# CHIANGEL/MAP-CODE

Measured on AMD Instinct MI355X. Metric: pretrain samples/sec (DCNv2+MFP, Avazu, bs4096), higher is better.
Workload: dtype f32; 1 GPU; DCNv2+MFP pretrain step, avazu-shaped synthetic ids (Zipf(1.1) per field), F=23, V=9449445, E=16, H=1000x3, cross x3, P=32, K=25, mask_ratio 0.3, fp32 GEMMs as three fp16 MFMAs per product (operands scaled by per-tensor magnitude records and cut into two fp16 pieces, fp32 accumulation; weights cut once per optimizer step); per_gpu_batch=4096, global_batch=4096, parallelism=dp1, launch=hipGraph replay of the whole step, table_optimizer=row-sparse AdamW with lazy replay of untouched rows, 400 untimed pre-roll steps

## Files before the change

### map-code_amd/csrc/amax.h

```cpp
#pragma once
#include "common.h"

namespace mapx {

typedef unsigned long long amax_rec;
constexpr int kAmaxSlots = 64;

const int32_t* amax_epoch_ptr();

__device__ inline uint32_t finite_abs_bits(float v) {
  const uint32_t u = __float_as_uint(v) & 0x7fffffffu;
  return u < 0x7f800000u ? u : 0u;
}
__device__ inline uint32_t amax4(uint32_t m, float a, float b, float c, float d) {
  const uint32_t x = max(finite_abs_bits(a), finite_abs_bits(b)), y = max(finite_abs_bits(c), finite_abs_bits(d));
  return max(m, max(x, y));
}
__device__ inline uint32_t wave_max_u32(uint32_t v) {
#pragma unroll
  for (int o = 32; o >= 1; o >>= 1) v = max(v, (uint32_t)__shfl_xor((int)v, o, kWave));
  return v;
}
__device__ inline int amax_slot() {
  return (int)(((blockIdx.x + blockIdx.y * gridDim.x + blockIdx.z * gridDim.x * gridDim.y) * (blockDim.x >> 6) +
                (threadIdx.x >> 6)) & (kAmaxSlots - 1));
}
__device__ inline void amax_publish(amax_rec* rec, uint32_t bits, const int32_t* epoch, int ahead = 0, int slot = 0) {
  const unsigned long long tag = epoch ? (unsigned long long)(uint32_t)(*epoch + ahead) : 0ull;
  atomicMax(rec + (slot & (kAmaxSlots - 1)), (tag << 32) | bits);
}
__device__ inline void amax_publish_wave(amax_rec* rec, uint32_t bits, const int32_t* epoch, int ahead = 0) {
  bits = wave_max_u32(bits);
  if ((threadIdx.x & 63) == 0) amax_publish(rec, bits, epoch, ahead, amax_slot());
}

__device__ inline void amax_publish_block(amax_rec* rec, uint32_t bits, const int32_t* epoch, int ahead = 0) {
  __shared__ uint32_t wave_bits[16];
  bits = wave_max_u32(bits);
  if ((threadIdx.x & 63) == 0) wave_bits[threadIdx.x >> 6] = bits;
  __syncthreads();
  if (threadIdx.x == 0) {
    uint32_t m = wave_bits[0];
    for (int w = 1; w < (int)(blockDim.x >> 6); ++w) m = max(m, wave_bits[w]);
    amax_publish(rec, m, epoch, ahead, (int)(blockIdx.x + blockIdx.y * gridDim.x + blockIdx.z * gridDim.x * gridDim.y));
  }
  __syncthreads();
}

__device__ inline uint32_t amax_read(const float* rec) {
  if (!rec) return 0u;
  return wave_max_u32(reinterpret_cast<const uint32_t*>(rec)[2 * (threadIdx.x & 63)] & 0x7fffffffu);
}
__device__ inline int h2_scale_exp(const float* rec) {
  const uint32_t b = amax_read(rec);
  const int e = (int)(b >> 23);
  if (b == 0u || e == 255) return 0;
  int n = 14 - (e - 127);
  return n > 126 ? 126 : (n < -126 ? -126 : n);
}
__device__ inline float pow2f(int n) { return __uint_as_float((uint32_t)(n + 127) << 23); }

}
```

### map-code_amd/csrc/gemm.hip

```cpp
#include "../../include/mapx_hip.h"
#include "common.h"
#include "amax.h"
#include "gemm_grouped.h"
#include "gemm_x3_common.h"

namespace mapx {


constexpr int kLayoutMaxT = 96 * 1024;

constexpr int kLayoutMwThreads = 1024;
constexpr int kLayoutBatch = 8;
__global__ void __launch_bounds__(kLayoutMwThreads) enc_group_layout_mw_kernel(
    const int64_t* __restrict__ masked_index, int T, int L, int F, int cap_slots, int32_t* __restrict__ rowmap,
    int32_t* __restrict__ hpos, int32_t* __restrict__ tile_group, int32_t* __restrict__ group_start) {
  constexpr int NW = kLayoutMwThreads / 64;
  __shared__ int hist[64];
  __shared__ int wave_match[NW];
  __shared__ int gs[64 + 1];
  extern __shared__ uint8_t fld[];
  const int f = blockIdx.x;
  const int lane = threadIdx.x & 63, wave = threadIdx.x >> 6;
  if (threadIdx.x < 64) hist[threadIdx.x] = 0;
  __syncthreads();
// ... 282 lines not shown
}

extern "C" int mapx_gemm_f32_batched(int count, int a_kc, int b_kc, int M, int N, int K, const float* const* A,
                                     int64_t lda, const float* const* B, int64_t ldb, float* const* C, int nsplit,
                                     void* ws, size_t ws_bytes, const mapx_gemm_scale* scales_opt,
                                     hipStream_t stream) {
  using namespace mapx;
  MAPX_REQUIRE(count >= 1 && count <= 4 && A && B && C, "gemm_f32_batched: 1 to 4 problems");
  MAPX_REQUIRE(M > 0 && N > 0 && K > 0, "gemm_f32_batched: empty problem");
  MAPX_REQUIRE(!(a_kc == 0 && b_kc != 0), "gemm_f32_batched: layout (A m-contiguous, B k-contiguous) unused");
  if (nsplit < 1) nsplit = 1;
  GemmX3Extra ex{};
  ex.batch = count;
  for (int z = 0; z < count; ++z) {
    MAPX_REQUIRE(A[z] && B[z] && C[z], "gemm_f32_batched: null operand");
    ex.Az[z] = A[z]; ex.Bz[z] = B[z]; ex.Cz[z] = C[z];
    if (scales_opt) { ex.amax_az[z] = scales_opt[z].amax_a; ex.amax_bz[z] = scales_opt[z].amax_b; }
  }
  if (count == 1) {
    ex.amax_a = ex.amax_az[0]; ex.amax_b = ex.amax_bz[0];
    return gemm_f32x3_launch(a_kc, b_kc, M, N, K, A[0], lda, B[0], ldb, C[0], N, MAPX_EPI_NONE, nullptr, nullptr, 0,
                             nullptr, 0, nullptr, 0, nsplit, -1, ws, ws_bytes, nullptr, stream, &ex);
  }
  int got = 0;
  for (int z = 1; z < count; ++z)
    MAPX_REQUIRE(((uintptr_t)A[z] % 16 == 0) == ((uintptr_t)A[0] % 16 == 0) &&
                     ((uintptr_t)B[z] % 16 == 0) == ((uintptr_t)B[0] % 16 == 0),
                 "gemm_f32_batched: operands of one launch must share their alignment");
  const int st = gemm_f32x3_launch(a_kc, b_kc, M, N, K, A[0], lda, B[0], ldb, C[0], N, MAPX_EPI_NONE, nullptr, nullptr, 0,
                                   nullptr, 0, nullptr, 0, nsplit, -1, ws, ws_bytes, &got, stream, &ex);
  if (st != MAPX_OK) return st;
  if (got > 1) {
    SumTasks t;
    memset(&t, 0, sizeof(t));
    for (int z = 0; z < count; ++z) {
      t.t[z].dst = C[z];
      t.t[z].src = static_cast<const float*>(ws) + (int64_t)z * nsplit * M * N;
      t.t[z].stride = (int64_t)M * N; t.t[z].n = (int64_t)M * N; t.t[z].nsplit = got;
    }
    hipLaunchKernelGGL(sum_tasks_kernel, dim3(96, count), dim3(256), 0, stream, t);
  }
  return check_launch("gemm_f32_batched");
}

extern "C" int mapx_enc_group_layout(const int64_t* masked_index, int T, int L, int F, int cap_slots,
                                     int32_t* rowmap, int32_t* hpos, int32_t* tile_group,
                                     int32_t* group_start, hipStream_t stream) {
  using namespace mapx;
  MAPX_REQUIRE(masked_index && rowmap && hpos && tile_group && group_start, "enc_group_layout: null pointer");
  MAPX_REQUIRE(F >= 1 && F <= 64 && L >= 1 && T >= 0 && cap_slots % 128 == 0 && cap_slots >= T + 127 * F,
               "enc_group_layout: bad sizes (F <= 64, cap_slots multiple of 128 and >= T + 127 F)");
  MAPX_REQUIRE(T <= kLayoutMaxT, "enc_group_layout: at most %d targets per step", kLayoutMaxT);
  const size_t dyn = ((size_t)T + 15) & ~(size_t)15;
  static bool raised = false;
  if (!raised) {
    MAPX_HIP(hipFuncSetAttribute(reinterpret_cast<const void*>(&enc_group_layout_mw_kernel),
                                 hipFuncAttributeMaxDynamicSharedMemorySize, kLayoutMaxT));
    raised = true;
  }
  hipLaunchKernelGGL(enc_group_layout_mw_kernel, dim3(F), dim3(kLayoutMwThreads), dyn, stream, masked_index, T, L, F,
                     cap_slots, rowmap, hpos, tile_group, group_start);
  return check_launch("enc_group_layout");
}

extern "C" int mapx_enc_grouped_fwd(const float* final_act, int64_t ld_final, int nrows, int K, const float* W,
                                    int64_t ldw, const float* bias, const int32_t* rowmap,
                                    const int32_t* tile_group, const int32_t* group_start_opt, int F,
                                    int cap_slots, float* h_slots, float* zero_slots_opt,
                                    const mapx_gemm_scale* scale_opt, hipStream_t stream) {
  using namespace mapx;
  MAPX_REQUIRE(final_act && W && bias && rowmap && tile_group && h_slots, "enc_grouped_fwd: null pointer");
  MAPX_REQUIRE(K % 4 == 0 && ld_final % 4 == 0 && ldw % 4 == 0 && cap_slots % 128 == 0,
               "enc_grouped_fwd: K, leading dimensions %% 4 and cap_slots %% 128 must be 0");
  GroupedArgs g{};
  g.A = final_act; g.lda = ld_final; g.B = W; g.ldb = ldw; g.C = h_slots; g.ldc = 32; g.bias = bias;
  g.rowmap = rowmap; g.tile_group = tile_group; g.K = K; g.N = 32; g.nrows = nrows;
  g.group_start = group_start_opt; g.F = F;
  g.zero_out = zero_slots_opt;
  MAPX_REQUIRE(K % 8 == 0 && ld_final % 4 == 0 && ldw % 4 == 0 && (uintptr_t)final_act % 16 == 0 && (uintptr_t)W % 16 == 0,
               "enc_grouped_fwd: K %% 8 != 0 or operands not 16-byte aligned (use the dense encoder GEMM)");
  static const bool h2 = [] { const char* e = getenv("MAPX_GEMM_H2"); return !e || atoi(e) != 0; }();
  if (h2 && scale_opt && scale_opt->amax_a && scale_opt->amax_b) {
    g.amax_a = scale_opt->amax_a; g.amax_b = scale_opt->amax_b;
    MAPX_HIP(enc_grouped_fwd_h2_launch(g, cap_slots, stream));
  } else {
    MAPX_HIP(enc_grouped_fwd_x3_launch(g, cap_slots, stream));
  }
  return check_launch("enc_grouped_fwd");
}

extern "C" int mapx_enc_grouped_dw(const float* dh_slots, const float* final_act, int64_t ld_final, int nrows,
                                   int N, const int32_t* rowmap, const int32_t* group_start, int F,
                                   const float* gscale_opt, float* dW, int64_t ldw, const mapx_gemm_scale* scale_opt,
                                   hipStream_t stream) {
  using namespace mapx;
  MAPX_REQUIRE(dh_slots && final_act && rowmap && group_start && dW, "enc_grouped_dw: null pointer");
  MAPX_REQUIRE(N % 4 == 0 && ld_final % 4 == 0 && F >= 1, "enc_grouped_dw: N, ld %% 4 must be 0");
  GroupedArgs g{};
  g.A = dh_slots; g.lda = 32; g.B = final_act; g.ldb = ld_final; g.C = dW; g.ldc = ldw;
  g.rowmap = rowmap; g.group_start = group_start; g.F = F; g.K = 0; g.N = N; g.nrows = nrows;
  g.gscale = gscale_opt;
  MAPX_REQUIRE(N % 8 == 0 && (uintptr_t)final_act % 16 == 0 && (uintptr_t)dh_slots % 16 == 0,
               "enc_grouped_dw: N %% 8 != 0 or operands not 16-byte aligned (use the dense encoder GEMM)");
  static const bool h2 = [] { const char* e = getenv("MAPX_GEMM_H2"); return !e || atoi(e) != 0; }();
  if (h2 && scale_opt && scale_opt->amax_a && scale_opt->amax_b) {
    g.amax_a = scale_opt->amax_a; g.amax_b = scale_opt->amax_b;
    MAPX_HIP(enc_grouped_dw_h2_launch(g, F, stream));
  } else {
    MAPX_HIP(enc_grouped_dw_x3_launch(g, F, stream));
  }
  return check_launch("enc_grouped_dw");
}

extern "C" size_t mapx_colsum_workspace_bytes(int N) {
  return (size_t)mapx::kColChunks * N * sizeof(float);
}

extern "C" int mapx_sum_tasks(const mapx_sum_task* tasks_host, int ntasks, hipStream_t stream) {
  using namespace mapx;
  MAPX_REQUIRE(ntasks >= 0 && ntasks <= kMaxSumTasks, "sum_tasks: at most %d tasks per call", kMaxSumTasks);
  if (ntasks == 0) return MAPX_OK;
  MAPX_REQUIRE(tasks_host, "sum_tasks: null task list");
  SumTasks t;
  memset(&t, 0, sizeof(t));
  for (int i = 0; i < ntasks; ++i) {
    MAPX_REQUIRE(tasks_host[i].dst && tasks_host[i].src && tasks_host[i].nsplit >= 1 && tasks_host[i].n >= 0,
                 "sum_tasks: bad task %d", i);
    t.t[i] = tasks_host[i];
  }
  hipLaunchKernelGGL(sum_tasks_kernel, dim3(96, ntasks), dim3(256), 0, stream, t);
  return check_launch("sum_tasks");
}

extern "C" int mapx_colsum_chunks(void) { return mapx::kColChunks; }

extern "C" int mapx_colsum(const float* x, int64_t ld, int M, int N, float* out, void* ws,
                           size_t ws_bytes, hipStream_t stream) {
  using namespace mapx;
  MAPX_REQUIRE(x && M >= 0 && N > 0, "colsum: bad arguments");
  if (!ws || ws_bytes < mapx_colsum_workspace_bytes(N)) {
    set_error("colsum: workspace too small");
    return MAPX_EWORKSPACE;
  }
  float* part = static_cast<float*>(ws);
  hipLaunchKernelGGL(colsum_stage1_kernel, dim3((N + 63) / 64, kColChunks), dim3(256), 0, stream, x,
                     ld, M, N, part);
  if (out)
    hipLaunchKernelGGL(colsum_stage2_kernel, dim3((N + 255) / 256), dim3(256), 0, stream, part, N, out);
  return check_launch("colsum");
}

extern "C" int mapx_relu_mask_colsum(const float* dy, int64_t ld_dy, const float* y, int64_t ld_y, int M, int N,
                                     float* dz, float* db, void* ws, size_t ws_bytes, void* amax_out_opt,
                                     hipStream_t stream) {
  using namespace mapx;
  MAPX_REQUIRE(dy && y && dz && M >= 0 && N > 0, "relu_mask_colsum: bad arguments");
  MAPX_REQUIRE(N % 4 == 0 && ld_dy % 4 == 0 && ld_dy >= N && (uintptr_t)dy % 16 == 0 && ld_y % 4 == 0 &&
                   ld_y >= N && (uintptr_t)y % 16 == 0,
               "relu_mask_colsum: N, ld_dy, ld_y %% 4 != 0 or dy / y not 16-byte aligned");
  if (!ws || ws_bytes < mapx_colsum_workspace_bytes(N)) {
    set_error("relu_mask_colsum: workspace too small");
    return MAPX_EWORKSPACE;
  }
  float* part = static_cast<float*>(ws);
  if (ew_narrow_lanes(N))
    hipLaunchKernelGGL((ew_colsum_kernel<0, 32>), dim3((N + 127) / 128, kColChunks), dim3(256), 0, stream, dy, ld_dy, y,
// ... 42 lines not shown
```

### map-code_amd/csrc/gemm_grouped.h

```cpp
#pragma once
#include <cstdint>
#include <hip/hip_runtime.h>

namespace mapx {

struct GroupedArgs {
  const float* A; int64_t lda;
  const float* B; int64_t ldb;
  float* C; int64_t ldc;
  const float* bias;
  const int32_t* rowmap;
  const int32_t* tile_group;
  const int32_t* group_start;
  int F;
  int K, N, nrows;
  float* zero_out;
  const float* gscale;
  const float* amax_a;
  const float* amax_b;
};

hipError_t enc_grouped_fwd_x3_launch(const GroupedArgs& g, int cap_slots, hipStream_t stream);
hipError_t enc_grouped_dw_x3_launch(const GroupedArgs& g, int F, hipStream_t stream);
hipError_t enc_grouped_fwd_h2_launch(const GroupedArgs& g, int cap_slots, hipStream_t stream);
hipError_t enc_grouped_dw_h2_launch(const GroupedArgs& g, int F, hipStream_t stream);

#ifdef __HIPCC__
__device__ inline int grouped_fwd_tile(const GroupedArgs& a, int lane, int wave) {
  constexpr int BM = 128;
  int tile = blockIdx.x;
  if (a.group_start) {
    const int used = a.group_start[a.F] / BM, per = (used + 7) / 8;
    if ((int)gridDim.x >= 8 * per && a.F <= 64) {
      const int i = blockIdx.x / 8, pos = (blockIdx.x % 8) * per + i;
      if (i >= per || pos >= used) return -1;
      __shared__ int below[8];
      const int gs0 = lane < a.F ? a.group_start[lane] : 0, gs1 = lane < a.F ? a.group_start[lane + 1] : 0;
      const int nf = (gs1 - gs0) / BM;
      int v = (wave * nf + 7) >> 3;
#pragma unroll
      for (int d = 32; d >= 1; d >>= 1) v += __shfl_xor(v, d);
      if (lane == 0) below[wave] = v;
      __syncthreads();
      int X = 0;
#pragma unroll
      for (int x = 1; x < 8; ++x)
        if (below[x] <= pos) X = x;
      const int q = pos - below[X];
      const int j0 = (X * nf + 7) >> 3, c = (((X + 1) * nf + 7) >> 3) - j0;
      int incl = c;
#pragma unroll
      for (int d = 1; d < 64; d <<= 1) {
        const int u = __shfl_up(incl, d);
        if (lane >= d) incl += u;
      }
      const bool hit = q >= incl - c && q < incl;
      const unsigned long long m = __ballot(hit);
      if (m == 0) return -1;
      tile = __shfl(gs0 / BM + j0 + (q - (incl - c)), __ffsll((long long)m) - 1);
    }
  }
  return tile;
}

#endif

}
```

### map-code_amd/csrc/gemm_grouped_h2.hip

```cpp
#include "gemm_grouped.h"
#include "gemm_h2_common.h"

namespace mapx {

template <bool DW>
__global__ void __launch_bounds__(512) gemm_grouped_h2_kernel(GroupedArgs a) {
  constexpr int NT = 512;
  constexpr int BM = DW ? 32 : 128, BN = DW ? 128 : 32;
  using OpA = OperandH2<BM, 1, !DW, NT>;
  using OpB = OperandH2<BN, 1, !DW, NT>;
  static_assert(OpA::NV == 1 && OpB::NV == 1, "one chunk per thread per operand");
  extern __shared__ __attribute__((aligned(16))) unsigned char smem_raw[];
  f16_t* const smem = reinterpret_cast<f16_t*>(smem_raw);
  const int na = __builtin_amdgcn_readfirstlane(h2_scale_exp(a.amax_a));
  const int nb = __builtin_amdgcn_readfirstlane(h2_scale_exp(a.amax_b));
  const float sA = pow2f(na), sB = pow2f(nb);
  const int dn = -(na + nb);
  constexpr int kBuf = OpA::LDS_ELEMS + OpB::LDS_ELEMS;
  const int lane = threadIdx.x & 63, wave = threadIdx.x >> 6;
  const int l31 = lane & 31, kh = lane >> 5;
  const int w4 = wave & 3, half = wave >> 2;
  const int abase = DW ? 0 : w4 * 32, bbase = DW ? w4 * 32 : 0;

  int f, kbeg, kend, n0 = 0, slot0 = 0;
  if (DW) {
    const int nb = gridDim.x, per = nb / 8;
    int lin = blockIdx.x;
    if (lin < per * 8) lin = (lin % 8) * per + lin / 8;
    f = lin % a.F;
    n0 = (lin / a.F) * BN;
    kbeg = a.group_start[f];
    kend = a.group_start[f + 1];
  } else {
    if (a.zero_out) {
      float4* z = reinterpret_cast<float4*>(a.zero_out + (int64_t)blockIdx.x * BM * 32);
      for (int i = threadIdx.x; i < BM * 32 / 4; i += NT) z[i] = make_float4(0.f, 0.f, 0.f, 0.f);
    }
    const int tile = grouped_fwd_tile(a, lane, wave);
    if (tile < 0) return;
    f = a.tile_group[tile];
    if (f < 0) return;
    slot0 = tile * BM;
    kbeg = 0;
    kend = a.K;
  }
  const float* __restrict__ Bb = DW ? a.B : a.B + (int64_t)f * 32 * a.ldb;

  f32x16 acc, cor;
#pragma unroll
  for (int r = 0; r < 16; ++r) acc[r] = cor[r] = 0.f;

  int atr, atc, btr, btc;
  OpA::coords(threadIdx.x, atr, atc);
  OpB::coords(threadIdx.x, btr, btc);
  const bool a_mine = !OpA::PARTIAL || threadIdx.x < OpA::TOTAL;
  const bool b_mine = !OpB::PARTIAL || threadIdx.x < OpB::TOTAL;
  int64_t arow = 0;
  bool arow_ok = false;
  if (!DW) {
    const int row = a.rowmap[slot0 + atr];
    arow_ok = row >= 0;
    arow = (int64_t)(row >= 0 ? row : 0) * a.lda + atc;
  }
  OpA la[2];
  OpB lb[2];
  int bnext = -1;
#define MAPX_GX_ROW(t) (DW ? ((kbeg + (t) * kXBK + btr) < kend ? a.rowmap[kbeg + (t) * kXBK + btr] : -1) : 0)
#define MAPX_GX_LOAD(SET, t, BROW)                                                                   \
  do {                                                                                               \
    const int k0 = kbeg + (t) * kXBK;                                                                \
    if (a_mine) {                                                                                    \
      const float* q;                                                                                \
      if (DW) {                                                                                      \
        la[SET].ok[0] = (k0 + atr) < kend;                                                           \
        q = a.A + (la[SET].ok[0] ? (int64_t)(k0 + atr) * a.lda + atc : 0);                           \
      } else {                                                                                       \
        la[SET].ok[0] = arow_ok && (k0 + atc) < kend;                                                \
        q = a.A + (la[SET].ok[0] ? arow + k0 : 0);                                                   \
      }                                                                                              \
      la[SET].r[0][0] = *reinterpret_cast<const float4*>(q);                                         \
      la[SET].r[0][1] = *reinterpret_cast<const float4*>(q + 4);                                     \
    }                                                                                                \
    if (b_mine) {                                                                                    \
      const float* q;                                                                                \
      if (DW) {                                                                                      \
        const int row = (BROW);                                                                      \
        lb[SET].ok[0] = row >= 0 && (n0 + btc) < a.N;                                                \
        q = Bb + (lb[SET].ok[0] ? (int64_t)row * a.ldb + n0 + btc : 0);                              \
      } else {                                                                                       \
        lb[SET].ok[0] = (k0 + btc) < kend;                                                           \
        q = Bb + (int64_t)btr * a.ldb + (lb[SET].ok[0] ? k0 + btc : 0);                              \
      }                                                                                              \
      lb[SET].r[0][0] = *reinterpret_cast<const float4*>(q);                                         \
      lb[SET].r[0][1] = *reinterpret_cast<const float4*>(q + 4);                                     \
    }                                                                                                \
  } while (0)
#define MAPX_GX_STORE(SET, buf)                                                                      \
  do {                                                                                               \
    la[SET].store_masked(smem + (buf) * kBuf, sA);                                                   \
    lb[SET].store_masked(smem + (buf) * kBuf + OpA::LDS_ELEMS, sB);                                  \
  } while (0)
  const int nk = (kend - kbeg + kXBK - 1) / kXBK;
  if (nk > 0) MAPX_GX_LOAD(0, 0, MAPX_GX_ROW(0));
  if (nk > 1) MAPX_GX_LOAD(1, 1, MAPX_GX_ROW(1));
  if (nk > 0) MAPX_GX_STORE(0, 0);
  if (nk > 2) MAPX_GX_LOAD(0, 2, MAPX_GX_ROW(2));
  if (nk > 3) bnext = MAPX_GX_ROW(3);
  __syncthreads();
#define MAPX_GX_KSTEP(CUR, kt, STEADY)                                                               \
  do {                                                                                               \
    const f16_t* const As_cur = smem + (CUR) * kBuf;                                                 \
    const f16_t* const Bs_cur = As_cur + OpA::LDS_ELEMS;                                             \
    const f16x8 ah = OpA::frag1(As_cur, 0, abase, lane, half, 0), bh = OpB::frag1(Bs_cur, 0, bbase, lane, half, 0); \
    const f16x8 al = OpA::frag1(As_cur, 1, abase, lane, half, 0), bl = OpB::frag1(Bs_cur, 1, bbase, lane, half, 0); \
    cor = __builtin_amdgcn_mfma_f32_32x32x16_f16(al, bh, cor, 0, 0, 0);                              \
    cor = __builtin_amdgcn_mfma_f32_32x32x16_f16(ah, bl, cor, 0, 0, 0);                              \
    acc = __builtin_amdgcn_mfma_f32_32x32x16_f16(ah, bh, acc, 0, 0, 0);                              \
    if ((STEADY) || (kt) + 1 < nk) MAPX_GX_STORE((CUR) ^ 1, (CUR) ^ 1);                              \
     \
     \
    int bnew = -1;                                                                                   \
    if (DW && ((STEADY) || (kt) + 4 < nk)) bnew = MAPX_GX_ROW((kt) + 4);                             \
    if ((STEADY) || (kt) + 3 < nk) MAPX_GX_LOAD((CUR) ^ 1, (kt) + 3, bnext);                         \
    bnext = bnew;                                                                                    \
    __syncthreads();                                                                                 \
  } while (0)
  int kt = 0;
  for (; kt + 5 < nk; kt += 2) {
    MAPX_GX_KSTEP(0, kt, true);
    MAPX_GX_KSTEP(1, kt + 1, true);
  }
  for (; kt < nk; kt += 2) {
    MAPX_GX_KSTEP(0, kt, false);
    if (kt + 1 < nk) MAPX_GX_KSTEP(1, kt + 1, false);
  }
#undef MAPX_GX_KSTEP
#undef MAPX_GX_STORE
#undef MAPX_GX_LOAD
#undef MAPX_GX_ROW

  float* const part = reinterpret_cast<float*>(smem_raw);
  if (half == 1) {
#pragma unroll
    for (int r = 0; r < 16; ++r) part[(w4 * 16 + r) * 64 + lane] = __builtin_fmaf(cor[r], 0x1p-11f, acc[r]);
  }
  __syncthreads();
  if (half == 1) return;
  const int n = (DW ? n0 : 0) + bbase + l31;
  if (DW ? (n < a.N) : true) {
    const float bn = DW ? 0.f : a.bias[f * 32 + n];
    const float gs = (DW && a.gscale) ? *a.gscale : 1.f;
    float* __restrict__ Cb = DW ? a.C + (int64_t)f * 32 * a.ldc : a.C + (int64_t)slot0 * a.ldc;
#pragma unroll
    for (int r = 0; r < 16; ++r) {
      const int m = abase + (r & 3) + 8 * (r >> 2) + 4 * kh;
      const float v = __builtin_ldexpf(__builtin_fmaf(cor[r], 0x1p-11f, acc[r]) + part[(w4 * 16 + r) * 64 + lane], dn);
      Cb[(int64_t)m * a.ldc + n] = DW ? v * gs : v + bn;
    }
  }
}


template <bool DW>
static hipError_t launch_grouped_h2(const GroupedArgs& g, dim3 grid, hipStream_t stream) {
  constexpr int BM = DW ? 32 : 128, BN = DW ? 128 : 32;
  using OpA = OperandH2<BM, 1, !DW, 512>;
  using OpB = OperandH2<BN, 1, !DW, 512>;
  constexpr size_t lds = (size_t)2 * (OpA::LDS_ELEMS + OpB::LDS_ELEMS) * sizeof(f16_t);
  static_assert(lds >= 4 * 16 * 64 * sizeof(float) && lds <= 160 * 1024, "LDS budget");
  auto* fn = &gemm_grouped_h2_kernel<DW>;
  static hipError_t raised =
      hipFuncSetAttribute(reinterpret_cast<const void*>(fn), hipFuncAttributeMaxDynamicSharedMemorySize, (int)lds);
  if (raised != hipSuccess) return raised;
  hipLaunchKernelGGL(fn, grid, dim3(512), lds, stream, g);
  return hipSuccess;
}

hipError_t enc_grouped_fwd_h2_launch(const GroupedArgs& g, int cap_slots, hipStream_t stream) {
  return launch_grouped_h2<false>(g, dim3(cap_slots / 128), stream);
}
hipError_t enc_grouped_dw_h2_launch(const GroupedArgs& g, int F, hipStream_t stream) {
  return launch_grouped_h2<true>(g, dim3(((g.N + 127) / 128) * F), stream);
}

}
```

### map-code_amd/csrc/gemm_h2w.hip

```cpp
#include "amax.h"
#include "gemm_x3_common.h"

namespace mapx {

typedef _Float16 f16_t;
typedef _Float16 f16x8 __attribute__((ext_vector_type(8)));
typedef uint32_t u32x4 __attribute__((ext_vector_type(4)));

constexpr int kPlaneHeader = 256;

struct CutRegs {
  float sx[4], r[4];
};
__device__ __forceinline__ void w_unit0(float x0a, float x1a, float x0b, float x1b, float s, CutRegs& c) {
  asm volatile("v_mul_f32 %0, %8, %4\n\t"
               "v_mul_f32 %1, %8, %5\n\t"
               "v_mul_f32 %2, %8, %6\n\t"
               "v_mul_f32 %3, %8, %7"
               : "=&v"(c.sx[0]), "=&v"(c.sx[1]), "=&v"(c.sx[2]), "=&v"(c.sx[3])
               : "v"(x0a), "v"(x1a), "v"(x0b), "v"(x1b), "s"(s));
}
__device__ __forceinline__ void w_unit1(CutRegs& c, uint32_t& Ha, uint32_t& Hb) {
  asm volatile("v_cvt_pk_f16_f32 %0, %4, %5\n\t"
               "v_cvt_pk_f16_f32 %1, %6, %7\n\t"
               "v_fma_mix_f32 %2, %4, 1.0, -%0 op_sel:[0,0,0] op_sel_hi:[0,0,1]\n\t"
               "v_fma_mix_f32 %3, %6, 1.0, -%1 op_sel:[0,0,0] op_sel_hi:[0,0,1]"
               : "=&v"(Ha), "=&v"(Hb), "=&v"(c.r[0]), "=&v"(c.r[2])
               : "v"(c.sx[0]), "v"(c.sx[1]), "v"(c.sx[2]), "v"(c.sx[3]));
}
__device__ __forceinline__ void w_unit2(CutRegs& c, uint32_t Ha, uint32_t Hb, float k2048) {
  asm volatile("v_fma_mix_f32 %0, %4, 1.0, -%6 op_sel:[0,0,1] op_sel_hi:[0,0,1]\n\t"
               "v_fma_mix_f32 %1, %5, 1.0, -%7 op_sel:[0,0,1] op_sel_hi:[0,0,1]\n\t"
               "v_mul_f32 %2, %8, %2\n\t"
               "v_mul_f32 %3, %8, %3"
               : "=&v"(c.r[1]), "=&v"(c.r[3]), "+v"(c.r[0]), "+v"(c.r[2])
               : "v"(c.sx[1]), "v"(c.sx[3]), "v"(Ha), "v"(Hb), "s"(k2048));
}
__device__ __forceinline__ void w_unit3(CutRegs& c, float k2048, uint32_t& La, uint32_t& Lb) {
  asm volatile("v_mul_f32 %2, %4, %2\n\t"
               "v_mul_f32 %3, %4, %3\n\t"
               "v_cvt_pk_f16_f32 %0, %5, %2\n\t"
               "v_cvt_pk_f16_f32 %1, %6, %3"
               : "=&v"(La), "=&v"(Lb), "+v"(c.r[1]), "+v"(c.r[3])
               : "s"(k2048), "v"(c.r[0]), "v"(c.r[2]));
}
__device__ inline void w_cut8(const float (&x)[8], float s, uint4& hi, uint4& lo) {
  uint32_t H[4], L[4];
#pragma unroll
  for (int e = 0; e < 4; e += 2) {
    CutRegs c;
    w_unit0(x[2 * e], x[2 * e + 1], x[2 * e + 2], x[2 * e + 3], s, c);
    w_unit1(c, H[e], H[e + 1]);
    w_unit2(c, H[e], H[e + 1], 2048.f);
    w_unit3(c, 2048.f, L[e], L[e + 1]);
  }
  hi = make_uint4(H[0], H[1], H[2], H[3]);
  lo = make_uint4(L[0], L[1], L[2], L[3]);
}

__global__ void __launch_bounds__(256) h2_weight_planes_kernel(const float* __restrict__ W, int64_t ldw, int N, int K,
                                                               int b_kc, const float* __restrict__ amax,
                                                               unsigned char* __restrict__ planes) {
  const int KS = ((K + 31) / 32) * 2, NT32 = (N + 31) / 32;
  const int lane = threadIdx.x & 63, r = lane & 31, h = lane >> 5;
  const int n_exp = h2_scale_exp(amax);
  const float s = pow2f(n_exp);
  if (blockIdx.x == 0 && threadIdx.x == 0) *reinterpret_cast<int32_t*>(planes) = n_exp;
  const int64_t blocks = (int64_t)NT32 * KS;
  for (int64_t blk = (int64_t)blockIdx.x * 4 + (threadIdx.x >> 6); blk < blocks; blk += (int64_t)gridDim.x * 4) {
    const int t = (int)(blk / KS), sidx = (int)(blk % KS);
    const int n = 32 * t + r, k0 = 16 * sidx + 8 * h;
    float x[8];
#pragma unroll
    for (int j = 0; j < 8; ++j) {
      const int k = k0 + j;
      const bool in = n < N && k < K;
      x[j] = in ? (b_kc ? W[(int64_t)n * ldw + k] : W[(int64_t)k * ldw + n]) : 0.f;
    }
    uint4 hi, lo;
    w_cut8(x, s, hi, lo);
    unsigned char* dst = planes + kPlaneHeader + blk * 2048 + lane * 16;
    *reinterpret_cast<uint4*>(dst) = hi;
    *reinterpret_cast<uint4*>(dst + 1024) = lo;
  }
}

constexpr int kMaxPlaneTasks = 16;
struct PlaneTasks {
  mapx_plane_task t[kMaxPlaneTasks];
  int64_t first[kMaxPlaneTasks + 1];
  int n;
};
// ... 595 lines not shown
```

### map-code_amd/mapx/ops.py

```python
import math
import os

import torch

import ctypes

from . import native as N
from .native import check, lib, ptr, require_gpu, stream


def native_int():
    return ctypes.c_int(0)


def native_byref(x):
    return ctypes.byref(x)

_scratch = {}
_scratch_retired = []

_timers = None


class Timers:
# ... 554 lines not shown
    return packed


def alias_draw(packed, targets, K, seed, offset, offset_dev=None):
    require_gpu(packed, targets)
    targets = targets.contiguous()
    T = targets.numel()
    idx = torch.empty(T, K + 1, dtype=torch.int32, device=targets.device)
    check(lib.mapx_alias_draw(ptr(packed), packed.shape[0], ptr(targets), T, K, seed, offset,
                              ptr(offset_dev), ptr(idx), stream()))
    return idx


def nce_pack_idx(targets, noise, V, validate=False):
    require_gpu(targets, noise)
    targets, noise = targets.contiguous(), noise.contiguous()
    T, K = targets.numel(), noise.shape[-1]
    idx = torch.empty(T, K + 1, dtype=torch.int32, device=targets.device)
    err = _err_flag(targets.device) if validate else None
    check(lib.mapx_nce_pack_idx(ptr(targets), ptr(noise), T, K, V, ptr(idx), ptr(err), stream()))
    if validate and int(err.item()):
        raise IndexError("index out of range in self")
    return idx


def lazy_rows_supported(P, K1):
    return P == 32 and K1 <= 32


def nce_fwd(enc, masked_index, idx, emb, bias, logq, F, P, want_logits=False, hpos=None, dh_slots=None,
            totals_later=False, lazy=None):
    require_gpu(enc, masked_index, idx, emb, bias, logq)
    B, L = masked_index.shape
    T, K1 = idx.shape
    assert T == B * L and (hpos is not None or enc.shape == (B, F * P))
    dev = enc.device
    f32 = dict(dtype=torch.float32, device=dev)
    out = dict(loss=torch.empty(2, **f32), acc=torch.empty(1, dtype=torch.int32, device=dev),
               h=torch.empty(T, P, **f32), dlogit=torch.empty(T, K1, **f32),
               dh=torch.empty(T, P, **f32),
               logits=torch.empty(T, K1, **f32) if want_logits else None)
    nws = lib.mapx_nce_fwd_workspace_bytes()
    ws = torch.empty(nws, dtype=torch.uint8, device=dev) if totals_later else scratch(nws, dev)
    left = native_int() if totals_later else None
    rec = amax_record(dev) if (dh_slots is not None and P == 32 and K1 <= 32) else None
    with _timed("nce_fwd", T * K1 * (4.0 * P + 8 + 4)):
        check(lib.mapx_nce_fwd(ptr(enc), B, L, F, P, ptr(masked_index.contiguous()), ptr(idx), K1 - 1,
                               ptr(emb), ptr(bias), ptr(logq), emb.shape[0], ptr(out["h"]),
                               ptr(out["dlogit"]), ptr(out["dh"]), ptr(out["logits"]), ptr(out["loss"]),
                               ptr(out["acc"]), ptr(ws), ws.numel(), ptr(hpos), ptr(dh_slots),
                               None if left is None else native_byref(left), ptr(rec),
                               None if lazy is None else native_byref(lazy), stream()))
    tag(dh_slots, rec)
    tag(out["dh"], rec)
    out["totals"] = (ws, left.value, out["loss"], out["acc"]) if (left is not None and left.value > 0) else None
    return out


class EncGroups:

    def __init__(self, masked_index, F):
        require_gpu(masked_index)
        B, L = masked_index.shape
        T, dev = B * L, masked_index.device
        self.T, self.L, self.F = T, L, F
        self.cap = (T + 127 * F + 1023) // 1024 * 1024
        masked_index = masked_index.contiguous()
        i32 = dict(dtype=torch.int32, device=dev)
        self.rowmap = torch.empty(self.cap, **i32)
        self.hpos = torch.empty(T, **i32)
        self.tile_group = torch.empty(self.cap // 128, **i32)
        self.group_start = torch.empty(F + 1, **i32)
        check(lib.mapx_enc_group_layout(ptr(masked_index), T, L, F, self.cap, ptr(self.rowmap), ptr(self.hpos),
                                        ptr(self.tile_group), ptr(self.group_start), stream()))


def _enc_groups_tensors(self):
    return (self.rowmap, self.hpos, self.tile_group, self.group_start)


EncGroups.tensors = _enc_groups_tensors


def enc_grouped_fwd(final, w, b, groups, zero_slots=None):
    require_gpu(final, w, b)
    h = torch.empty(groups.cap, 32, dtype=torch.float32, device=final.device)
    ra, rb = amax_of(final), amax_of(w)
    if AUTO_AMAX and H2:
        ra = ra if ra is not None else amax(final)
        rb = rb if rb is not None else amax(w)
    sc = _scale_arg(ra, rb) if (ra is not None and rb is not None) else None
    with _timed("gemm_enc_grouped_fwd", 2.0 * groups.T * 32 * final.shape[1]):
        check(lib.mapx_enc_grouped_fwd(final.data_ptr(), final.stride(0), final.shape[0], final.shape[1],
                                       ptr(w), w.stride(0), ptr(b), ptr(groups.rowmap), ptr(groups.tile_group),
                                       ptr(groups.group_start), groups.F, groups.cap, ptr(h), ptr(zero_slots),
                                       None if sc is None else native_byref(sc), stream()))
    return h


def enc_grouped_dw(dh_slots, final, groups, out=None, gscale=None):
    require_gpu(dh_slots, final)
    Nn = final.shape[1]
    if out is None:
        out = torch.empty(groups.F * 32, Nn, dtype=torch.float32, device=final.device)
    ra, rb = amax_of(dh_slots), amax_of(final)
    if AUTO_AMAX and H2:
        ra = ra if ra is not None else amax(dh_slots)
        rb = rb if rb is not None else amax(final)
    sc = _scale_arg(ra, rb) if (ra is not None and rb is not None) else None
    with _timed("gemm_enc_grouped_dw", 2.0 * groups.T * 32 * Nn):
        check(lib.mapx_enc_grouped_dw(ptr(dh_slots), final.data_ptr(), final.stride(0), final.shape[0], Nn,
                                      ptr(groups.rowmap), ptr(groups.group_start), groups.F, ptr(gscale),
                                      ptr(out), out.stride(0), None if sc is None else native_byref(sc), stream()))
    return out


def nce_scatter_dh(dh, masked_index, F, P, gscale=None, totals=None):
    require_gpu(dh, masked_index)
    B, L = masked_index.shape
    denc = torch.empty(B, F * P, dtype=torch.float32, device=dh.device)
    ws, n, loss, acc = totals if totals is not None else (None, 0, None, None)
    rec = amax_record(dh.device)
    check(lib.mapx_nce_scatter_dh(ptr(dh), ptr(masked_index.contiguous()), ptr(gscale), B, L, F, P,
                                  ptr(denc), ptr(ws), n, ptr(loss), ptr(acc), ptr(rec), stream()))
    return tag(denc, rec)


def nce_table_grad(plan, dlogit, h, K, P, gscale=None):
    dev = dlogit.device
    out_emb = torch.empty(max(plan.n, 1), P, dtype=torch.float32, device=dev)
    out_bias = torch.empty(max(plan.n, 1), dtype=torch.float32, device=dev)
    nb = lib.mapx_nce_table_grad_workspace_bytes(plan.n, P)
    ws = scratch(nb, dev)
    with _timed("nce_table_grad", plan.n * (4.0 * P + 4)):
        check(lib.mapx_nce_table_grad(plan.n, ptr(plan.perm), ptr(plan.rank), ptr(plan.seg_start),
                                      ptr(dlogit), ptr(h), K, P, ptr(gscale), ptr(out_emb), ptr(out_bias),
                                      ptr(ws), ws.numel(), plan.take_counter(), stream()))
    return out_emb, out_bias


def scale_(x, g):
    check(lib.mapx_scale_inplace(ptr(x), x.numel(), ptr(g), stream()))
    return x


_EPI_RELU_MASK_COLSUM = N.EPI_RELU_MASK_COLSUM


def gemm_bf16(a, b, a_kc, b_kc, M, N, K, out=None, out_dtype=BF16, ldc=None, epi=N.EPI_NONE, bias=None,
              aux1=None, aux2=None, out2=None, nsplit=1, lda=None, ldb=None, tile=-1):
    require_gpu(a, b)
    if not (is_bf16(a) and is_bf16(b)):
        raise TypeError("gemm_bf16 takes bf16 operands")
    dev = a.device
    if out is None:
        out = torch.empty(M, N, dtype=out_dtype, device=dev)
    c_f32 = out.dtype == torch.float32
    if not (c_f32 or is_bf16(out)):
        raise TypeError("gemm_bf16 writes bf16 or fp32")
    ldc = ldc if ldc is not None else out.stride(0)
    lda = lda if lda is not None else a.stride(0)
    ldb = ldb if ldb is not None else b.stride(0)
    ws, wsn = None, 0
    if nsplit > 1:
        wsn = lib.mapx_gemm_splitk_workspace_bytes(M, N, nsplit)
        ws = scratch(wsn, dev)
        wsn = ws.numel()
    if bias is not None and bias.dtype != torch.float32:
        raise TypeError("gemm_bf16: the bias stays fp32")
    aux1_f32 = aux1 is not None and aux1.dtype == torch.float32
    for t_ in (aux2, out2):
        if t_ is not None and not is_bf16(t_) and not (t_ is out2 and epi == _EPI_RELU_MASK_COLSUM):
            raise TypeError("gemm_bf16: aux2 / out2 are bf16 (out2 of EPI_RELU_MASK_COLSUM: fp32 partial rows)")
    kind = "gemm_fwd_nt" if (a_kc and b_kc) else ("gemm_dx_nn" if a_kc else "gemm_dw_tn")
# ... 95 lines not shown

def amax_pack(*ts):
    return tuple(amax_of(t) for t in ts)


def amax_unpack(ts, recs):
    for t, r in zip(ts, recs):
        tag(t, r)


def out_record(out, device):
    rec = amax_of(out)
    return rec if rec is not None else amax_record(device)


def amax(x, rec=None, reset=True):
    require_gpu(x)
    if x.dtype != torch.float32:
        raise TypeError("amax: fp32 tensors")
    _ensure_epoch(x.device)
    if rec is None:
        rec = torch.empty(REC, dtype=torch.int32, device=x.device)
        reset = True
    x2 = x if x.dim() == 2 else x.reshape(1, -1)
    if x2.stride(1) != 1:
        x2 = x2.contiguous()
    check(lib.mapx_amax_f32(x2.data_ptr(), x2.shape[0], x2.shape[1], x2.stride(0), rec.data_ptr(), int(reset), stream()))
    return rec


def amax_value(rec):
    return float(rec[0::2].max().view(1).view(torch.float32).item())


AMAX_CHECK = os.environ.get("MAPX_AMAX_CHECK", "0") == "1"
AUTO_AMAX = os.environ.get("MAPX_AUTO_AMAX", "0") == "1"
H2_USED = [0, 0]


def _check_record(x, rec, what):
    if rec is None:
        return
    xs = x.detach().float()
    xs = xs[torch.isfinite(xs)]
    true = float(xs.abs().max()) if xs.numel() else 0.0
    got = amax_value(rec)
    if not (got >= true and (true == 0.0 or got <= true * 64.0 or got < 1e-30)):
        raise AssertionError(f"magnitude record of operand {what}: {got!r} for a tensor whose max |x| is {true!r}")


H2W = os.environ.get("MAPX_GEMM_H2W", "1") == "1"


def h2_weight_planes(w, b_kc, rec, out=None):
    require_gpu(w)
    Nn, K = (w.shape[0], w.shape[1]) if b_kc else (w.shape[1], w.shape[0])
    if out is None:
        out = torch.empty(lib.mapx_h2_weight_planes_bytes(Nn, K), dtype=torch.uint8, device=w.device)
    check(lib.mapx_h2_weight_planes(w.data_ptr(), w.stride(0), Nn, K, int(b_kc), rec.data_ptr(), out.data_ptr(), stream()))
    return out


def planes_wanted(M, Nn, K):
    return math.ceil(M / 128) * math.ceil(Nn / 64) >= 128 and K >= 64 and K % 8 == 0


def weight_planes(w, b_kc, M):
    if not (H2 and H2W) or w is None or w.dim() != 2 or w.dtype != torch.float32:
        return None
    base, c0, c1 = getattr(w, "_wslice", (w, 0, None))
    reg = getattr(base, "_planes", None)
    rec = amax_of(base)
    if reg is None or rec is None:
        return None
    Nn, K = (w.shape[0], w.shape[1]) if b_kc else (w.shape[1], w.shape[0])
    if not planes_wanted(M, Nn, K):
        return None
    key = (bool(b_kc), c0, c1)
    pl = reg.get(key)
    if pl is None:
        if torch.cuda.is_current_stream_capturing():
            return None
        pl = reg[key] = h2_weight_planes(base.detach()[:, c0:c1] if (c0, c1) != (0, None) else base.detach(), b_kc, rec)
    return pl


def refresh_weight_planes(params):
    if isinstance(params, torch.Tensor):
        params = [params]
    todo = []
    for p in params:
        for (b_kc, c0, c1), pl in (getattr(p, "_planes", None) or {}).items():
            w = p.detach()[:, c0:c1] if (c0, c1) != (0, None) else p.detach()
            Nn, K = (w.shape[0], w.shape[1]) if b_kc else (w.shape[1], w.shape[0])
            todo.append((w, Nn, K, b_kc, p._amax, pl))
    for i in range(0, len(todo), 16):
        part = todo[i:i + 16]
        arr = (N.PlaneTask * len(part))()
        for j, (w, Nn, K, b_kc, rec, pl) in enumerate(part):
            arr[j].W, arr[j].ldw, arr[j].N, arr[j].K, arr[j].b_kc = w.data_ptr(), w.stride(0), Nn, K, int(b_kc)
            arr[j].amax_record, arr[j].planes = rec.data_ptr(), pl.data_ptr()
        check(lib.mapx_h2_weight_planes_multi(arr, len(part), stream()))


def _as2d(t, ld):
    return t if t.dim() == 2 else t.reshape(-1, ld)


def _scale_arg(amax_a, amax_b, amax_c=None, amax_c2=None, b_planes=None):
    if amax_a is None and amax_b is None and amax_c is None and amax_c2 is None:
        return None
    sc = N.GemmScale()
    sc.b_planes = b_planes.data_ptr() if (b_planes is not None and amax_a is not None) else None
    sc.amax_a = amax_a.data_ptr() if amax_a is not None else None
    sc.amax_b = amax_b.data_ptr() if amax_b is not None else None
    sc.amax_c = amax_c.data_ptr() if amax_c is not None else None
    sc.amax_c2 = amax_c2.data_ptr() if amax_c2 is not None else None
    return sc


def gemm(a, b, a_kc, b_kc, M, N, K, out=None, ldc=None, epi=N.EPI_NONE, bias=None, aux1=None,
         aux2=None, out2=None, nsplit=1, lda=None, ldb=None, tile=-1, out_dtype=None,
         amax_a=None, amax_b=None, amax_c=None, record=True, b_planes=None):
    require_gpu(a, b)
    if is_bf16(a):
        return gemm_bf16(a, b, a_kc, b_kc, M, N, K, out=out, out_dtype=out_dtype or BF16, ldc=ldc, epi=epi,
                         bias=bias, aux1=aux1, aux2=aux2, out2=out2, nsplit=nsplit, lda=lda, ldb=ldb, tile=tile)
    dev = a.device
    if out is None:
        out = torch.empty(M, N, dtype=torch.float32, device=dev)
    ldc = ldc if ldc is not None else out.stride(0)
    lda = lda if lda is not None else a.stride(0)
    ldb = ldb if ldb is not None else b.stride(0)
    ws, wsn = None, 0
    if nsplit > 1:
        ws = scratch(lib.mapx_gemm_splitk_workspace_bytes(M, N, nsplit), dev)
        wsn = ws.numel()
    ld1 = aux1.stride(0) if aux1 is not None else 0
    ld2 = aux2.stride(0) if aux2 is not None else 0
    ldo2 = out2.stride(0) if out2 is not None else 0
    kind = "gemm_fwd_nt" if (a_kc and b_kc) else ("gemm_dx_nn" if a_kc else "gemm_dw_tn")
    amax_a = amax_a if amax_a is not None else amax_of(a)
    amax_b = amax_b if amax_b is not None else amax_of(b)
    if AUTO_AMAX and H2:
        amax_a = amax_a if amax_a is not None else amax(_as2d(a, lda))
        amax_b = amax_b if amax_b is not None else amax(_as2d(b, ldb))
        if b_planes is None and H2W and a_kc and nsplit == 1 and tile < 0 and planes_wanted(M, N, K) \
                and b.dim() == 2 and b.stride(1) == 1:
            b_planes = h2_weight_planes(b[:N, :K] if b_kc else b[:K, :N], b_kc, amax_b)
    if amax_c is None and record and nsplit == 1:
        amax_c = out_record(out, dev)
    H2_USED[0 if (amax_a is not None and amax_b is not None) else 1] += 1
    if AMAX_CHECK and not torch.cuda.is_current_stream_capturing():
        _check_record(a, amax_a, "A")
        _check_record(b, amax_b, "B")
    sc = _scale_arg(amax_a, amax_b, amax_c, b_planes=b_planes if b_planes is not None else
                    (weight_planes(b, b_kc, M) if (a_kc and nsplit == 1 and tile < 0) else None))
    with _timed(kind, 2.0 * M * N * K):
        check(lib.mapx_gemm_f32(int(a_kc), int(b_kc), M, N, K, a.data_ptr(), lda, b.data_ptr(), ldb,
                                out.data_ptr(), ldc, epi, ptr(bias),
                                aux1.data_ptr() if aux1 is not None else None, ld1,
                                aux2.data_ptr() if aux2 is not None else None, ld2,
                                out2.data_ptr() if out2 is not None else None, ldo2, nsplit, tile,
                                ws.data_ptr() if ws is not None else None, wsn, None,
                                None if sc is None else native_byref(sc), stream()))
    return tag(out, amax_c)
# ... 685 lines not shown
```

Baseline: 5.940 million samples/s.

## Feed grouped encoder forward GEMM from precut fp16 weight planes

The grouped encoder forward GEMM can now read the weight operand from precomputed fp16 hi/lo planes, which are cut once per optimizer step and cached. Fragments are loaded straight into registers instead of being cut from fp32, scaled and staged through LDS. This removes the per-tile weight conversion and halves LDS use for the B operand. The kernel is also restructured to process KS k-subtiles per pipeline stage. The cost is extra register pressure and a separate prefetch path, and it depends on plane registration having happened before graph capture.

```diff
diff --git a/map-code_amd/csrc/amax.h b/map-code_amd/csrc/amax.h
--- a/map-code_amd/csrc/amax.h
+++ b/map-code_amd/csrc/amax.h
@@ -60,4 +60,6 @@
 }
 __device__ inline float pow2f(int n) { return __uint_as_float((uint32_t)(n + 127) << 23); }
 
+constexpr int kPlaneHeader = 256;
+
 }
diff --git a/map-code_amd/csrc/gemm.hip b/map-code_amd/csrc/gemm.hip
--- a/map-code_amd/csrc/gemm.hip
+++ b/map-code_amd/csrc/gemm.hip
@@ -388,6 +388,10 @@
   static const bool h2 = [] { const char* e = getenv("MAPX_GEMM_H2"); return !e || atoi(e) != 0; }();
   if (h2 && scale_opt && scale_opt->amax_a && scale_opt->amax_b) {
     g.amax_a = scale_opt->amax_a; g.amax_b = scale_opt->amax_b;
+    if (scale_opt->b_planes) {
+      MAPX_REQUIRE((uintptr_t)scale_opt->b_planes % 16 == 0, "enc_grouped_fwd: planes must be 16-byte aligned");
+      g.b_planes = static_cast<const unsigned char*>(scale_opt->b_planes);
+    }
     MAPX_HIP(enc_grouped_fwd_h2_launch(g, cap_slots, stream));
   } else {
     MAPX_HIP(enc_grouped_fwd_x3_launch(g, cap_slots, stream));
diff --git a/map-code_amd/csrc/gemm_grouped.h b/map-code_amd/csrc/gemm_grouped.h
--- a/map-code_amd/csrc/gemm_grouped.h
+++ b/map-code_amd/csrc/gemm_grouped.h
@@ -18,6 +18,7 @@
   const float* gscale;
   const float* amax_a;
   const float* amax_b;
+  const unsigned char* b_planes;
 };
 
 hipError_t enc_grouped_fwd_x3_launch(const GroupedArgs& g, int cap_slots, hipStream_t stream);
diff --git a/map-code_amd/csrc/gemm_grouped_h2.hip b/map-code_amd/csrc/gemm_grouped_h2.hip
--- a/map-code_amd/csrc/gemm_grouped_h2.hip
+++ b/map-code_amd/csrc/gemm_grouped_h2.hip
@@ -3,20 +3,35 @@
 
 namespace mapx {
 
-template <bool DW>
-__global__ void __launch_bounds__(512) gemm_grouped_h2_kernel(GroupedArgs a) {
-  constexpr int NT = 512;
-  constexpr int BM = DW ? 32 : 128, BN = DW ? 128 : 32;
+#ifndef MAPX_GROUPED_KSUB_FWD
+#define MAPX_GROUPED_KSUB_FWD 2
+#endif
+#ifndef MAPX_GROUPED_KSUB_DW
+#define MAPX_GROUPED_KSUB_DW 2
+#endif
+
+typedef uint32_t u32x4 __attribute__((ext_vector_type(4)));
+
+template <bool DW, bool PL>
+struct GroupedH2 {
+  static_assert(!(DW && PL), "the weight gradient reads no weight");
+  static constexpr int NT = 512;
+  static constexpr int KS = DW ? MAPX_GROUPED_KSUB_DW : (PL || MAPX_GROUPED_KSUB_FWD <= 2 ? MAPX_GROUPED_KSUB_FWD : 2);
+  static constexpr int BM = DW ? 32 : 128, BN = DW ? 128 : 32;
   using OpA = OperandH2<BM, 1, !DW, NT>;
   using OpB = OperandH2<BN, 1, !DW, NT>;
-  static_assert(OpA::NV == 1 && OpB::NV == 1, "one chunk per thread per operand");
-  extern __shared__ __attribute__((aligned(16))) unsigned char smem_raw[];
+  static_assert(OpA::NV == 1 && OpB::NV == 1, "one chunk per thread per operand and sub-tile");
+  static constexpr int kSub = OpA::LDS_ELEMS + (PL ? 0 : OpB::LDS_ELEMS);
+  static constexpr int kBuf = KS * kSub;
+  static constexpr size_t kLds = (size_t)2 * kBuf * sizeof(f16_t);
+  static_assert(kLds >= 4 * 16 * 64 * sizeof(float) && kLds <= 160 * 1024, "LDS budget");
+
+  static __device__ __forceinline__ void run(const GroupedArgs& a, unsigned char* smem_raw) {
   f16_t* const smem = reinterpret_cast<f16_t*>(smem_raw);
   const int na = __builtin_amdgcn_readfirstlane(h2_scale_exp(a.amax_a));
-  const int nb = __builtin_amdgcn_readfirstlane(h2_scale_exp(a.amax_b));
+  const int nb = __builtin_amdgcn_readfirstlane(PL ? *reinterpret_cast<const int32_t*>(a.b_planes) : h2_scale_exp(a.amax_b));
   const float sA = pow2f(na), sB = pow2f(nb);
   const int dn = -(na + nb);
-  constexpr int kBuf = OpA::LDS_ELEMS + OpB::LDS_ELEMS;
   const int lane = threadIdx.x & 63, wave = threadIdx.x >> 6;
   const int l31 = lane & 31, kh = lane >> 5;
   const int w4 = wave & 3, half = wave >> 2;
@@ -45,6 +60,10 @@
     kend = a.K;
   }
   const float* __restrict__ Bb = DW ? a.B : a.B + (int64_t)f * 32 * a.ldb;
+  const int nk32 = (kend - kbeg + kXBK - 1) / kXBK;
+  const int nk = (nk32 + KS - 1) / KS;
+  const unsigned char* const pbase =
+      PL ? a.b_planes + kPlaneHeader + ((int64_t)f * 2 * nk32 + half) * 2048 + lane * 16 : nullptr;
 
   f32x16 acc, cor;
 #pragma unroll
@@ -54,7 +73,7 @@
   OpA::coords(threadIdx.x, atr, atc);
   OpB::coords(threadIdx.x, btr, btc);
   const bool a_mine = !OpA::PARTIAL || threadIdx.x < OpA::TOTAL;
-  const bool b_mine = !OpB::PARTIAL || threadIdx.x < OpB::TOTAL;
+  const bool b_mine = !PL && (!OpB::PARTIAL || threadIdx.x < OpB::TOTAL);
   int64_t arow = 0;
   bool arow_ok = false;
   if (!DW) {
@@ -62,67 +81,99 @@
     arow_ok = row >= 0;
     arow = (int64_t)(row >= 0 ? row : 0) * a.lda + atc;
   }
-  OpA la[2];
-  OpB lb[2];
-  int bnext = -1;
-#define MAPX_GX_ROW(t) (DW ? ((kbeg + (t) * kXBK + btr) < kend ? a.rowmap[kbeg + (t) * kXBK + btr] : -1) : 0)
+  OpA la[2][KS];
+  OpB lb[2][KS];
+  u32x4 fb[2][KS][2];
+  int bnext[KS], bnew[KS];
+#define MAPX_GX_ROWS(DST, t)                                                                         \
+  do {                                                                                               \
+  _Pragma("unroll") for (int j_ = 0; j_ < KS; ++j_) {                                                \
+    const int s_ = kbeg + ((t) * KS + j_) * kXBK + btr;                                              \
+    DST[j_] = (DW && s_ < kend) ? a.rowmap[s_] : -1;                                                 \
+  }                                                                                                  \
+  } while (0)
 #define MAPX_GX_LOAD(SET, t, BROW)                                                                   \
   do {                                                                                               \
-    const int k0 = kbeg + (t) * kXBK;                                                                \
+  _Pragma("unroll") for (int j_ = 0; j_ < KS; ++j_) {                                                \
+    const int k0 = kbeg + ((t) * KS + j_) * kXBK;                                                    \
     if (a_mine) {                                                                                    \
       const float* q;                                                                                \
       if (DW) {                                                                                      \
-        la[SET].ok[0] = (k0 + atr) < kend;                                                           \
-        q = a.A + (la[SET].ok[0] ? (int64_t)(k0 + atr) * a.lda + atc : 0);                           \
+        la[SET][j_].ok[0] = (k0 + atr) < kend;                                                       \
+        q = a.A + (la[SET][j_].ok[0] ? (int64_t)(k0 + atr) * a.lda + atc : 0);                       \
       } else {                                                                                       \
-        la[SET].ok[0] = arow_ok && (k0 + atc) < kend;                                                \
-        q = a.A + (la[SET].ok[0] ? arow + k0 : 0);                                                   \
+        la[SET][j_].ok[0] = arow_ok && (k0 + atc) < kend;                                            \
+        q = a.A + (la[SET][j_].ok[0] ? arow + k0 : 0);                                               \
       }                                                                                              \
-      la[SET].r[0][0] = *reinterpret_cast<const float4*>(q);                                         \
-      la[SET].r[0][1] = *reinterpret_cast<const float4*>(q + 4);                                     \
+      la[SET][j_].r[0][0] = *reinterpret_cast<const float4*>(q);                                     \
+      la[SET][j_].r[0][1] = *reinterpret_cast<const float4*>(q + 4);                                 \
     }                                                                                                \
     if (b_mine) {                                                                                    \
       const float* q;                                                                                \
       if (DW) {                                                                                      \
-        const int row = (BROW);                                                                      \
-        lb[SET].ok[0] = row >= 0 && (n0 + btc) < a.N;                                                \
-        q = Bb + (lb[SET].ok[0] ? (int64_t)row * a.ldb + n0 + btc : 0);                              \
+        const int row = (BROW)[j_];                                                                  \
+        lb[SET][j_].ok[0] = row >= 0 && (n0 + btc) < a.N;                                            \
+        q = Bb + (lb[SET][j_].ok[0] ? (int64_t)row * a.ldb + n0 + btc : 0);                          \
       } else {                                                                                       \
-        lb[SET].ok[0] = (k0 + btc) < kend;                                                           \
-        q = Bb + (int64_t)btr * a.ldb + (lb[SET].ok[0] ? k0 + btc : 0);                              \
+        lb[SET][j_].ok[0] = (k0 + btc) < kend;                                                       \
+        q = Bb + (int64_t)btr * a.ldb + (lb[SET][j_].ok[0] ? k0 + btc : 0);                          \
       }                                                                                              \
-      lb[SET].r[0][0] = *reinterpret_cast<const float4*>(q);                                         \
-      lb[SET].r[0][1] = *reinterpret_cast<const float4*>(q + 4);                                     \
+      lb[SET][j_].r[0][0] = *reinterpret_cast<const float4*>(q);                                     \
+      lb[SET][j_].r[0][1] = *reinterpret_cast<const float4*>(q + 4);                                 \
     }                                                                                                \
+  }                                                                                                  \
+  } while (0)
+#define MAPX_GX_BLOAD(SET, t)                                                                        \
+  do {                                                                                               \
+  _Pragma("unroll") for (int j_ = 0; j_ < KS; ++j_) {                                                \
+    const int s_ = (t) * KS + j_ < nk32 ? (t) * KS + j_ : nk32 - 1;                                  \
+    const unsigned char* const q_ = pbase + (int64_t)s_ * 4096;                                      \
+    fb[SET][j_][0] = *reinterpret_cast<const u32x4*>(q_);                                            \
+    fb[SET][j_][1] = *reinterpret_cast<const u32x4*>(q_ + 1024);                                     \
+  }                                                                                                  \
   } while (0)
 #define MAPX_GX_STORE(SET, buf)                                                                      \
   do {                                                                                               \
-    la[SET].store_masked(smem + (buf) * kBuf, sA);                                                   \
-    lb[SET].store_masked(smem + (buf) * kBuf + OpA::LDS_ELEMS, sB);                                  \
-  } while (0)
-  const int nk = (kend - kbeg + kXBK - 1) / kXBK;
-  if (nk > 0) MAPX_GX_LOAD(0, 0, MAPX_GX_ROW(0));
-  if (nk > 1) MAPX_GX_LOAD(1, 1, MAPX_GX_ROW(1));
+  _Pragma("unroll") for (int j_ = 0; j_ < KS; ++j_) {                                                \
+    if (a_mine) la[SET][j_].store_masked(smem + (buf) * kBuf + j_ * kSub, sA);                       \
+    if (b_mine) lb[SET][j_].store_masked(smem + (buf) * kBuf + j_ * kSub + OpA::LDS_ELEMS, sB);      \
+  }                                                                                                  \
+  } while (0)
+  if (nk > 0) { MAPX_GX_ROWS(bnext, 0); MAPX_GX_LOAD(0, 0, bnext); }
+  if (PL && nk > 0) MAPX_GX_BLOAD(0, 0);
+  if (nk > 1) { MAPX_GX_ROWS(bnext, 1); MAPX_GX_LOAD(1, 1, bnext); }
+  if (PL && nk > 1) MAPX_GX_BLOAD(1, 1);
   if (nk > 0) MAPX_GX_STORE(0, 0);
-  if (nk > 2) MAPX_GX_LOAD(0, 2, MAPX_GX_ROW(2));
-  if (nk > 3) bnext = MAPX_GX_ROW(3);
+  if (nk > 2) { MAPX_GX_ROWS(bnext, 2); MAPX_GX_LOAD(0, 2, bnext); }
+  MAPX_GX_ROWS(bnext, 3);
   __syncthreads();
 #define MAPX_GX_KSTEP(CUR, kt, STEADY)                                                               \
   do {                                                                                               \
-    const f16_t* const As_cur = smem + (CUR) * kBuf;                                                 \
-    const f16_t* const Bs_cur = As_cur + OpA::LDS_ELEMS;                                             \
-    const f16x8 ah = OpA::frag1(As_cur, 0, abase, lane, half, 0), bh = OpB::frag1(Bs_cur, 0, bbase, lane, half, 0); \
-    const f16x8 al = OpA::frag1(As_cur, 1, abase, lane, half, 0), bl = OpB::frag1(Bs_cur, 1, bbase, lane, half, 0); \
-    cor = __builtin_amdgcn_mfma_f32_32x32x16_f16(al, bh, cor, 0, 0, 0);                              \
-    cor = __builtin_amdgcn_mfma_f32_32x32x16_f16(ah, bl, cor, 0, 0, 0);                              \
-    acc = __builtin_amdgcn_mfma_f32_32x32x16_f16(ah, bh, acc, 0, 0, 0);                              \
+    _Pragma("unroll") for (int j_ = 0; j_ < KS; ++j_) {                                              \
+      if ((STEADY) || (kt) * KS + j_ < nk32) {                                                       \
+        const f16_t* const As_cur = smem + (CUR) * kBuf + j_ * kSub;                                 \
+        const f16_t* const Bs_cur = As_cur + OpA::LDS_ELEMS;                                         \
+        const f16x8 ah = OpA::frag1(As_cur, 0, abase, lane, half, 0), al = OpA::frag1(As_cur, 1, abase, lane, half, 0); \
+        f16x8 bh, bl;                                                                                \
+        if constexpr (PL) {                                                                          \
+          bh = __builtin_bit_cast(f16x8, fb[CUR][j_][0]);                                            \
+          bl = __builtin_bit_cast(f16x8, fb[CUR][j_][1]);                                            \
+        } else {                                                                                     \
+          bh = OpB::frag1(Bs_cur, 0, bbase, lane, half, 0);                                          \
+          bl = OpB::frag1(Bs_cur, 1, bbase, lane, half, 0);                                          \
+        }                                                                                            \
+        cor = __builtin_amdgcn_mfma_f32_32x32x16_f16(al, bh, cor, 0, 0, 0);                          \
+        cor = __builtin_amdgcn_mfma_f32_32x32x16_f16(ah, bl, cor, 0, 0, 0);                          \
+        acc = __builtin_amdgcn_mfma_f32_32x32x16_f16(ah, bh, acc, 0, 0, 0);                          \
+      }                                                                                              \
+    }                                                                                                \
     if ((STEADY) || (kt) + 1 < nk) MAPX_GX_STORE((CUR) ^ 1, (CUR) ^ 1);                              \
      \
      \
-    int bnew = -1;                                                                                   \
-    if (DW && ((STEADY) || (kt) + 4 < nk)) bnew = MAPX_GX_ROW((kt) + 4);                             \
+    MAPX_GX_ROWS(bnew, ((STEADY) || (kt) + 4 < nk) ? (kt) + 4 : nk);                                 \
+    if (PL && ((STEADY) || (kt) + 2 < nk)) MAPX_GX_BLOAD(CUR, (kt) + 2);                             \
     if ((STEADY) || (kt) + 3 < nk) MAPX_GX_LOAD((CUR) ^ 1, (kt) + 3, bnext);                         \
-    bnext = bnew;                                                                                    \
+    _Pragma("unroll") for (int j_ = 0; j_ < KS; ++j_) bnext[j_] = bnew[j_];                          \
     __syncthreads();                                                                                 \
   } while (0)
   int kt = 0;
@@ -136,8 +187,9 @@
   }
 #undef MAPX_GX_KSTEP
 #undef MAPX_GX_STORE
+#undef MAPX_GX_BLOAD
 #undef MAPX_GX_LOAD
-#undef MAPX_GX_ROW
+#undef MAPX_GX_ROWS
 
   float* const part = reinterpret_cast<float*>(smem_raw);
   if (half == 1) {
@@ -158,19 +210,30 @@
       Cb[(int64_t)m * a.ldc + n] = DW ? v * gs : v + bn;
     }
   }
+  }
+};
+
+template <bool DW>
+__global__ void __launch_bounds__(512) gemm_grouped_h2_kernel(GroupedArgs a) {
+  extern __shared__ __attribute__((aligned(16))) unsigned char smem_raw[];
+  if constexpr (DW) {
+    GroupedH2<true, false>::run(a, smem_raw);
+  } else {
+    if (a.b_planes) GroupedH2<false, true>::run(a, smem_raw);
+    else GroupedH2<false, false>::run(a, smem_raw);
+  }
 }
 
 
 template <bool DW>
 static hipError_t launch_grouped_h2(const GroupedArgs& g, dim3 grid, hipStream_t stream) {
-  constexpr int BM = DW ? 32 : 128, BN = DW ? 128 : 32;
-  using OpA = OperandH2<BM, 1, !DW, 512>;
-  using OpB = OperandH2<BN, 1, !DW, 512>;
-  constexpr size_t lds = (size_t)2 * (OpA::LDS_ELEMS + OpB::LDS_ELEMS) * sizeof(f16_t);
-  static_assert(lds >= 4 * 16 * 64 * sizeof(float) && lds <= 160 * 1024, "LDS budget");
+  constexpr size_t lds_max = DW ? GroupedH2<true, false>::kLds
+                                : (GroupedH2<false, false>::kLds > GroupedH2<false, true>::kLds ? GroupedH2<false, false>::kLds
+                                                                                                : GroupedH2<false, true>::kLds);
+  const size_t lds = DW ? GroupedH2<true, false>::kLds : (g.b_planes ? GroupedH2<false, true>::kLds : GroupedH2<false, false>::kLds);
   auto* fn = &gemm_grouped_h2_kernel<DW>;
   static hipError_t raised =
-      hipFuncSetAttribute(reinterpret_cast<const void*>(fn), hipFuncAttributeMaxDynamicSharedMemorySize, (int)lds);
+      hipFuncSetAttribute(reinterpret_cast<const void*>(fn), hipFuncAttributeMaxDynamicSharedMemorySize, (int)lds_max);
   if (raised != hipSuccess) return raised;
   hipLaunchKernelGGL(fn, grid, dim3(512), lds, stream, g);
   return hipSuccess;
diff --git a/map-code_amd/csrc/gemm_h2w.hip b/map-code_amd/csrc/gemm_h2w.hip
--- a/map-code_amd/csrc/gemm_h2w.hip
+++ b/map-code_amd/csrc/gemm_h2w.hip
@@ -6,8 +6,6 @@
 typedef _Float16 f16_t;
 typedef _Float16 f16x8 __attribute__((ext_vector_type(8)));
 typedef uint32_t u32x4 __attribute__((ext_vector_type(4)));
-
-constexpr int kPlaneHeader = 256;
 
 struct CutRegs {
   float sx[4], r[4];
diff --git a/map-code_amd/mapx/ops.py b/map-code_amd/mapx/ops.py
--- a/map-code_amd/mapx/ops.py
+++ b/map-code_amd/mapx/ops.py
@@ -660,14 +660,16 @@
 EncGroups.tensors = _enc_groups_tensors
 
 
-def enc_grouped_fwd(final, w, b, groups, zero_slots=None):
+def enc_grouped_fwd(final, w, b, groups, zero_slots=None, b_planes=None):
     require_gpu(final, w, b)
     h = torch.empty(groups.cap, 32, dtype=torch.float32, device=final.device)
     ra, rb = amax_of(final), amax_of(w)
     if AUTO_AMAX and H2:
         ra = ra if ra is not None else amax(final)
         rb = rb if rb is not None else amax(w)
-    sc = _scale_arg(ra, rb) if (ra is not None and rb is not None) else None
+    if b_planes is None:
+        b_planes = grouped_weight_planes(w)
+    sc = _scale_arg(ra, rb, b_planes=b_planes) if (ra is not None and rb is not None) else None
     with _timed("gemm_enc_grouped_fwd", 2.0 * groups.T * 32 * final.shape[1]):
         check(lib.mapx_enc_grouped_fwd(final.data_ptr(), final.stride(0), final.shape[0], final.shape[1],
                                        ptr(w), w.stride(0), ptr(b), ptr(groups.rowmap), ptr(groups.tile_group),
@@ -929,6 +931,26 @@
         if torch.cuda.is_current_stream_capturing():
             return None
         pl = reg[key] = h2_weight_planes(base.detach()[:, c0:c1] if (c0, c1) != (0, None) else base.detach(), b_kc, rec)
+    return pl
+
+
+def grouped_planes_wanted(w):
+    return (w.dim() == 2 and w.dtype == torch.float32 and w.stride(1) == 1 and w.shape[0] % 32 == 0
+            and w.shape[1] % 8 == 0 and w.data_ptr() % 16 == 0)
+
+
+def grouped_weight_planes(w):
+    if not (H2 and H2W) or w is None or hasattr(w, "_wslice") or not grouped_planes_wanted(w):
+        return None
+    reg, rec = getattr(w, "_planes", None), amax_of(w)
+    if reg is None or rec is None:
+        return None
+    key = (True, 0, None)
+    pl = reg.get(key)
+    if pl is None:
+        if torch.cuda.is_current_stream_capturing():
+            return None
+        pl = reg[key] = h2_weight_planes(w.detach(), True, rec)
     return pl
 
 
```

Result: slower. 5.798 million samples/s (-2.4%).
